# linkedin/spark-tfrecord

Measured on NVIDIA B200. Metric: TFRecord decode GB/s (1 KB Example, 64 mixed features) at 1/2/4/8 B200, higher is better.
Workload: dtype u8

## Files before the change

spark-tfrecord_b200/csrc/api_decode.inc:

```

static inline size_t align_up(size_t v, size_t a) { return (v + a - 1) / a * a; }

struct HostStats {
  FrameResult frame;
  DecodeSummary summary;
  uint32_t overflow;
  uint32_t pad[3];
};

struct K1Bufs {
  DevBuf chunks, chunk_base, first, stage, rec_off;
  uint32_t n_chunks = 0, chunk_bytes = 0;
  void release() { chunks.release(); chunk_base.release(); first.release(); stage.release(); rec_off.release(); }
};

struct PtrTables {
  void** h = nullptr; size_t cap = 0;
  DevBuf dev;
  int32_t ensure(size_t n_ptr) {
    if (cap < n_ptr) {
      if (h) cudaFreeHost(h);
      h = nullptr; cap = 0;
      CUDA_TRY(cudaHostAlloc((void**)&h, n_ptr * sizeof(void*), cudaHostAllocDefault));
      cap = n_ptr;
// ... 105 lines not shown
  unsigned long long* d_null_counts = nullptr;
  std::vector<unsigned long long> h_null_counts_tmp;
  void* host_copy = nullptr; size_t host_copy_bytes = 0;
  bool host_copy_enqueued = false;
  cudaEvent_t d2h_done = nullptr;
  bool null_counts_ready = false;
  cudaEvent_t done = nullptr;
  bool pending = false;
  Lane* lane = nullptr;
  const void* src = nullptr; size_t src_bytes = 0; int src_on_device = 0, is_final = 0;
  bool xc_tried = false;
  OutLayout lay;
  std::vector<size_t> lvl_off;
  std::vector<int32_t> uni_len;
};

static void give_event(tfr_decoder* d, cudaEvent_t e) { if (e) d->done_pool.push_back(e); }
static int32_t take_event(tfr_decoder* d, cudaEvent_t* e) {
  if (!d->done_pool.empty()) { *e = d->done_pool.back(); d->done_pool.pop_back(); return TFR_OK; }
  CUDA_TRY(cudaEventCreateWithFlags(e, cudaEventDisableTiming));
  return TFR_OK;
}

extern "C" int32_t tfr_decoder_create(const tfr_schema* schema, int32_t device, uint32_t flags, tfr_decoder** out) {
  if (!schema || !out) return fail(TFR_E_INVALID_ARG, "null argument");
  DeviceCtx* ctx = nullptr;
  int32_t rc = get_ctx(device, &ctx);
  if (rc) return rc;
  CUDA_TRY(cudaSetDevice(device));
  auto* d = new tfr_decoder;
  d->schema = *schema; d->device = device; d->flags = flags; d->ctx = ctx;
  CUDA_TRY(cudaStreamCreateWithFlags(&d->stream, cudaStreamNonBlocking));
  {
    int lo = 0, hi = 0;
    CUDA_TRY(cudaDeviceGetStreamPriorityRange(&lo, &hi));
    CUDA_TRY(cudaStreamCreateWithPriority(&d->st_k1, cudaStreamNonBlocking, getenv("TFR_NO_K1_PRIORITY") ? lo : hi));
  }
  CUDA_TRY(cudaStreamCreateWithFlags(&d->st_h2d, cudaStreamNonBlocking));
  CUDA_TRY(cudaStreamCreateWithFlags(&d->st_d2h, cudaStreamNonBlocking));
  CUDA_TRY(cudaStreamCreateWithFlags(&d->st_aux, cudaStreamNonBlocking));
  rc = d->dsch.upload(d->schema);
  if (!rc) rc = d->dsch.build_tile_consts(d->schema, ctx->d_tabs);
  if (rc) { delete d; return rc; }
  TRY(d->small.ensure(4096 + (size_t)d->schema.n_cnt * 16));
  {
    bool ok = d->schema.fields.size() <= 128 && !getenv("TFR_DISABLE_FAST");
    for (const DevField& f : d->schema.fields) if (f.depth > 1 && d->schema.record_type == TFR_RT_EXAMPLE) ok = false;
    d->fast_ok = ok;
    if (getenv("TFR_DISABLE_SPECULATION")) d->spec_state = -1;
    const size_t nv = std::max(1, d->schema.n_var);
    d->spec_len.assign(nv, -1);
    d->hist_ratio.assign(std::max(1, d->schema.n_cnt), 0.0);
    CUDA_TRY(cudaHostAlloc((void**)&d->h_uniform, nv * 4, cudaHostAllocDefault));
    TRY(d->uniform_dev.ensure(nv * 4));
    TRY(d->no_uniform_dev.ensure(nv * 4));
    CUDA_TRY(cudaMemset(d->no_uniform_dev.p, 0xff, nv * 4));
  }
  CUDA_TRY(cudaHostAlloc((void**)&d->h_stats, sizeof(HostStats), cudaHostAllocDefault));
  size_t nt = (size_t)d->schema.n_cnt * 2 + d->schema.fields.size() + 8;
  CUDA_TRY(cudaHostAlloc((void**)&d->h_totals, nt * sizeof(int64_t), cudaHostAllocDefault));
  for (Lane& L : d->lanes) {
    L.h_res_bytes = sizeof(LaneResult) + 8 * std::max<size_t>(1, d->schema.fields.size()) + 8 * std::max<size_t>(1, (size_t)d->schema.n_cnt);
    TRY(L.res.ensure(L.h_res_bytes));
    CUDA_TRY(cudaHostAlloc((void**)&L.h_res, L.h_res_bytes, cudaHostAllocDefault));
    CUDA_TRY(cudaEventCreateWithFlags(&L.ev_in, cudaEventDisableTiming));
    CUDA_TRY(cudaEventCreateWithFlags(&L.ev_k1, cudaEventDisableTiming));
    CUDA_TRY(cudaEventCreateWithFlags(&L.ev_tile, cudaEventDisableTiming));
    CUDA_TRY(cudaEventCreateWithFlags(&L.ev_frame, cudaEventDisableTiming));
    CUDA_TRY(cudaHostAlloc((void**)&L.h_frame, sizeof(FrameResult), cudaHostAllocDefault));
  }
  *out = d;
  return TFR_OK;
}
static void decoder_unref(tfr_decoder* d);
extern "C" void tfr_decoder_destroy(tfr_decoder* d) { if (d) decoder_unref(d); }
static void decoder_unref(tfr_decoder* d) {
  if (d->refs.fetch_sub(1) != 1) return;
  int prev = -1; cudaGetDevice(&prev);
  cudaSetDevice(d->device);
// ... 435 lines not shown
  return cudaSuccess;
}
static int32_t launch_bytes(DeviceCtx* ctx, const TileArgs& TA, uint32_t grid_rows, const TileGeom& g, cudaStream_t st) {
  const uint32_t grid = std::max<uint32_t>(1, (grid_rows + TILE_ROWS - 1) / TILE_ROWS);
  const size_t tiles_per_sm = std::max<size_t>(1, (size_t)233472 / (g.smem + 1024));
  static const int force = getenv("TFR_BYTES_CW") ? atoi(getenv("TFR_BYTES_CW")) : 0;
  const int cw = force ? force : tiles_per_sm >= 10 ? 4 : 8;
  cudaError_t e = cw <= 2 ? bytes_launch_one<2, 1>(ctx, TA, grid, g.smem, st) : cw <= 4 ? bytes_launch_one<4, 2>(ctx, TA, grid, g.smem, st) : bytes_launch_one<8, 4>(ctx, TA, grid, g.smem, st);
  if (e != cudaSuccess) return fail(TFR_E_CUDA, std::string("bytes kernel: ") + cudaGetErrorString(e));
  return TFR_OK;
}

static void batch_drop_outputs(tfr_batch* b) {
  tfr_decoder* d = b->dec;
  if (b->dev_fixed) { d->dev_pool.give_back(b->dev_fixed, d->stream); b->dev_fixed = nullptr; b->dev_fixed_bytes = 0; }
  if (b->dev_var) { d->dev_pool.give_back(b->dev_var, d->stream); b->dev_var = nullptr; b->dev_var_bytes = 0; }
  b->d_null_counts = nullptr; b->cols.clear(); b->null_counts_ready = false;
}

static int32_t decode_sync(tfr_decoder* d, tfr_batch* b, const void* data, size_t nbytes, int32_t data_on_device, int32_t is_final, bool allow_fast) {
  NvtxRange nvtx("tfr_decode_sync");
  cudaStream_t st = d->stream;
  const tfr_schema& S = d->schema;
  for (;;) {
    b->info = tfr_batch_info{};
    b->info.error_row = -1; b->info.error_field = -1;
    DecodeCtx C;
    C.d = d; C.b = b; C.st = st; C.nbytes = nbytes; C.nf = (uint32_t)S.fields.size(); C.lay = &b->lay; C.pt = &d->pt;
    C.verify = (d->flags & TFR_F_VERIFY_CRC) ? 1u : 0u;
    const uint32_t nf = C.nf;

    C.d_data = (const uint8_t*)data;
    if (!data_on_device && nbytes) {
      TRY(d->in.ensure(align_up(nbytes + 64, 256)));
      d->span_begin(5);
      CUDA_TRY(cudaMemcpyAsync(d->in.p, data, nbytes, cudaMemcpyHostToDevice, st));
      d->span_end(0);
      C.d_data = (const uint8_t*)d->in.p;
      data = d->in.p; data_on_device = 1;
    }
    const bool try_fast = allow_fast && d->fast_ok;
    const bool k1_verified = !try_fast || !C.verify;
    FrameResult fr{};
    fr.stop = FS_EOF;
    if (nbytes) {
      d->span_begin(0);
// ... 94 lines not shown
        TA.verify = C.verify; TA.names_bytes = names_bytes; TA.sch = d->dsch.view; TA.consts = d->dsch.d_tile_consts; TA.const_bytes = d->dsch.tile_consts_bytes;
        TA.bitmaps = C.fx + b->lay.bitmaps_off; TA.nb_stride = b->lay.nb_stride; TA.null_counts = b->d_null_counts;
        TA.fix_values = A.fix_values; TA.cnt = A.cnt; TA.src = A.src; TA.cflag = A.cflag;
        TA.uniform_len = (const int32_t*)(uniform ? d->uniform_dev.p : d->no_uniform_dev.p); TA.var_values = (void* const*)C.dt_vals; TA.flags = dflags_ptr(d);
        d->span_begin(1);
        TRY(launch_tile(d, TA, n, geom, st));
        d->span_end(1); d->pass1_launches++;
        uint32_t tflags = 0;
        if (uniform) {
          if (S.n_var) {
            d->span_begin(2);
            uniform_offsets_kernel<<<dim3(std::min<uint32_t>((n + 256) / 256, 512), S.n_var), 256, 0, st>>>((int32_t* const*)C.dt_offs, 3, (const int32_t*)d->uniform_dev.p, (uint32_t)S.n_var, n, nullptr);
            d->span_end(1);
          }
          CUDA_TRY(cudaMemcpyAsync(&d->h_stats->overflow, dovf_ptr(d), 8, cudaMemcpyDeviceToHost, st));
          CUDA_TRY(cudaStreamSynchronize(st));
          CUDA_TRY(cudaGetLastError());
          tflags = (&d->h_stats->overflow)[1];
          if (!(tflags & TF_FALLBACK)) {
            for (int a = 0; a < S.n_cnt; ++a) totals[a] = utot[a];
            TRY(finish_var_and_views(C, A, n, totals, false, false));
            done = true;
          } else {
            if (tflags & TF_SHAPE) {
              d->spec_state = 0;
              if (++d->shape_misses >= 2) d->relearn_backoff = 8;
            }
            if (b->dev_var) { d->dev_pool.give_back(b->dev_var, d->stream); b->dev_var = nullptr; b->dev_var_bytes = 0; }
            if (tflags & TF_SHAPE) {
              CUDA_TRY(cudaMemsetAsync(b->d_null_counts, 0, sizeof(unsigned long long) * std::max<uint32_t>(nf, 1), st));
              CUDA_TRY(cudaMemsetAsync(dflags_ptr(d), 0, 4, st));
              TA.uniform_len = (const int32_t*)d->no_uniform_dev.p;
              d->span_begin(1);
              TRY(launch_tile(d, TA, n, geom, st));
              d->span_end(1); d->pass1_launches++;
            }
          }
        }
        if (!done && (!uniform || (tflags & TF_SHAPE))) {
          TRY(scans_and_sync(C, A, false));
          tflags = (&d->h_stats->overflow)[1];
          if (!(tflags & TF_FALLBACK)) {
            if (d->h_stats->overflow)
              for (int a = 0; a < S.n_cnt; ++a) if (totals[a] < 0 || totals[a] > 0x7fffffffLL) return fail(TFR_E_BATCH_TOO_LARGE, "Arrow int32 offsets overflow; decode smaller blocks");
            A.flist_warp = S.record_type == TFR_RT_SEQUENCE_EXAMPLE && !getenv("TFR_DISABLE_FLIST_WARP");
            TRY(finish_var_and_views(C, A, n, totals, true, false));
            done = true;
            d->stats[3]++;
            if (d->relearn_backoff > 0) --d->relearn_backoff;
            else if (d->spec_state == 0) {
              bool ok = true, ragged = false;
              for (int v = 0; v < S.n_var && ok; ++v) {
                const DevField& fd = S.fields[S.var_field[v]];
                const int64_t c0 = totals[S.n_cnt + fd.cnt_slot];
                if (fd.n_levels == 1 && c0 > 0 && totals[fd.cnt_slot] == c0 * (int64_t)n) d->spec_len[v] = (int32_t)c0;
                else if (getenv("TFR_DISABLE_RAGGED")) ok = false;
                else if (fd.depth <= 1) { d->spec_len[v] = TILE_RAGGED; ragged = true; }
                else if (S.record_type == TFR_RT_SEQUENCE_EXAMPLE && S.n_var <= 4 && fd.elem_type != TFR_T_STRING && fd.elem_type != TFR_T_BINARY) {
                  d->spec_len[v] = TILE_RAGGED; ragged = true;
                } else ok = false;
              }
              if (ragged && ((size_t)tile_ragged_bytes((uint32_t)S.n_var, (uint32_t)S.n_cnt) > 24576 || S.n_cnt > 128)) ok = false;
              if (ok) {
                d->spec_state = 1; d->spec_ragged = ragged; d->stats[5]++;
                memcpy(d->h_uniform, d->spec_len.data(), (size_t)S.n_var * 4);
                CUDA_TRY(cudaMemcpyAsync(d->uniform_dev.p, d->h_uniform, (size_t)S.n_var * 4, cudaMemcpyHostToDevice, st));
                CUDA_TRY(cudaStreamSynchronize(st));
              }
            }
            for (int a = 0; a < S.n_cnt; ++a) d->hist_ratio[a] = used ? (double)totals[a] / (double)used : 0.0;
          }
        }
        if (done) { n_eff = n; sum.n_eff = n; if (uniform && !(tflags & TF_FALLBACK)) d->shape_misses = 0; }
      }
      if (!done && !k1_verified) {
        batch_drop_outputs(b);
        allow_fast = false;
        again = true;
      } else if (!done) {
        CUDA_TRY(cudaMemsetAsync(b->d_null_counts, 0, sizeof(unsigned long long) * std::max<uint32_t>(nf, 1), st));
        TRY(ensure_rec_off(C));
        fill_decode_args(C, A);
        const uint32_t warps = 8;
        size_t smem1 = CRC_SMEM_WORDS * 4 + (size_t)warps * ((nf + 3) & ~3u);
        uint32_t g1 = std::min<uint32_t>((n + warps - 1) / warps, (uint32_t)d->ctx->sm_count * 16);
        d->span_begin(1);
        decode_pass1_kernel<<<g1, warps * 32, smem1, st>>>(A);
        d->span_end(1); d->pass1_launches++;
        TRY(scans_and_sync(C, A, true));
// ... 9 lines not shown
      b->cols.resize(nf);
      for (uint32_t f = 0; f < nf; ++f) {
        const DevField& fd = S.fields[f];
        tfr_column c{};
        c.elem_type = fd.elem_type; c.depth = fd.depth; c.n_levels = fd.n_levels; c.value_width = fd.width;
        c.validity = C.fx + b->lay.bitmaps_off + (size_t)f * b->lay.nb_stride;
        if (fd.var_slot >= 0) { c.offsets[0] = (int32_t*)(C.fx + b->lay.off0_off[fd.var_slot]); c.n_offsets[0] = 1; }
        if (fd.fix_slot >= 0) c.values = C.fx + b->lay.fix_off[fd.fix_slot];
        for (int l = 1; l < fd.n_levels; ++l) { c.offsets[l] = c.offsets[0]; c.n_offsets[l] = 1; }
        b->cols[f] = c;
      }
    }
    if (again) continue;
    b->info.consumed_bytes = (int64_t)used;
    b->info.n_rows = n_eff;
    if (n > 0 && sum.first_err_row != 0xffffffffu) {
      b->info.error_code = -(int32_t)(sum.first_err_status & 0xff);
      b->info.error_row = sum.first_err_row;
      b->info.error_field = (int32_t)(sum.first_err_status >> 8) - 1;
    } else if (frame_err) {
      b->info.error_code = frame_err; b->info.error_row = n; b->info.error_field = -1;
    }
    if (!b->info.error_code && n > 64) { d->mean_rec_bytes = (double)fr.stop_pos / n; d->last_max_len = fr.max_len; d->last_max_tile = 0; }
    if (!b->done) TRY(take_event(d, &b->done));
    CUDA_TRY(cudaEventRecord(b->done, st));
    CUDA_TRY(cudaGetLastError());
    d->stats[0]++;
    return TFR_OK;
  }
}

static bool can_speculate(const tfr_decoder* d, const void* data, size_t nbytes, int32_t on_device, uint32_t* cap_out) {
  if (!d->fast_ok || d->spec_state != 1 || d->mean_rec_bytes < 16.0 || d->last_max_len == 0 || nbytes < 4096 || getenv("TFR_DISABLE_ASYNC")) return false;
  const double est = (double)nbytes / d->mean_rec_bytes;
  uint64_t cap = (uint64_t)(est * (1.0 + (getenv("TFR_FIXED_SLACK") ? 0.0625 : d->cap_slack))) + (getenv("TFR_FIXED_SLACK") ? 4096 : 1024);
  cap = std::min<uint64_t>(cap, nbytes / 16 + 1);
  for (int v = 0; v < d->schema.n_var; ++v) if (d->spec_len[v] >= 0 && (uint64_t)d->spec_len[v] * cap > 0x7fffffffull) return false;
  const uint32_t rg = (d->spec_ragged ? tile_ragged_bytes((uint32_t)d->schema.n_var, (uint32_t)d->schema.n_cnt) : 0u) +
                      (d->schema.record_type == TFR_RT_SEQUENCE_EXAMPLE ? tile_seq_bytes((uint32_t)d->schema.n_var, d->spec_ragged) : 0u);
  if (d->schema.record_type == TFR_RT_BYTE_ARRAY) { if (bytes_geom_for(d, d->last_max_len, true).smem > (size_t)d->ctx->max_smem_optin) return false; }
  else if (tile_geom_for(d, d->last_max_len, true, rg, d->last_max_tile).smem > (size_t)d->ctx->max_smem_optin) return false;
  *cap_out = (uint32_t)cap;
  return true;
}

static int32_t submit_async(tfr_decoder* d, Lane& L, tfr_batch* b, const void* data, size_t nbytes, int32_t on_device, int32_t is_final, uint32_t cap) {
// ... 169 lines not shown
    b->xc_tried = true;
    d->xc_batches = 64;
    const uint32_t cap = b->lay.n_alloc;
    batch_drop_outputs(b);
    b->host_copy_enqueued = false; b->host_cols.clear();
    if (b->d2h_done) CUDA_TRY(cudaEventSynchronize(b->d2h_done));
    if (b->host_copy) { d->host_pool.give_back(b->host_copy); b->host_copy = nullptr; }
    d->stats[6]++;
    TRY(submit_async(d, L, b, b->src, b->src_bytes, 1, b->is_final, cap));
    return resolve(b);
  }
  d->stats[2]++;
  if (fr.n_records > b->lay.n_alloc) d->cap_slack = 0.0625;
  const bool unlearned = (r.flags & TF_SHAPE) && d->spec_state == 1;
  if (r.flags & TF_SHAPE) {
    d->spec_state = 0;
    if (++d->shape_misses >= 2) d->relearn_backoff = 8;
  }
  batch_drop_outputs(b);
  b->host_copy_enqueued = false; b->host_cols.clear();
  if (b->d2h_done) CUDA_TRY(cudaEventSynchronize(b->d2h_done));
  if (b->host_copy) { d->host_pool.give_back(b->host_copy); b->host_copy = nullptr; }
  TRY(decode_sync(d, b, b->src, b->src_bytes, 1, b->is_final, true));
  if (b->src == L.in.p) CUDA_TRY(cudaEventSynchronize(b->done));
  if (unlearned && b->info.error_code && d->spec_state == 0) { d->spec_state = 1; if (d->shape_misses > 0) --d->shape_misses; d->relearn_backoff = 0; }
  return TFR_OK;
}

static int32_t lane_make_free(tfr_decoder* d, Lane& L) {
  if (L.pending) TRY(resolve(L.pending));
  if (L.orphan_done) {
    CUDA_TRY(cudaEventSynchronize(L.orphan_done));
    give_event(d, L.orphan_done); L.orphan_done = nullptr;
    const LaneResult r = *L.h_res;
    if (r.flags & TF_FALLBACK) d->stats[2]++;
    if (r.flags & TF_SHAPE) { d->spec_state = 0; if (++d->shape_misses >= 2) d->relearn_backoff = 8; }
    else if (!(r.flags & TF_FALLBACK) && r.frame.n_records > 64) { d->mean_rec_bytes = (double)r.frame.stop_pos / r.frame.n_records; d->last_max_len = r.frame.max_len; d->last_max_tile = r.max_tile; }
  }
  return TFR_OK;
}

extern "C" int32_t tfr_decode_submit(tfr_decoder* d, const void* data, size_t nbytes, int32_t data_on_device, int32_t is_final, tfr_batch** out) {
  if (!d || !out || (nbytes && !data)) return fail(TFR_E_INVALID_ARG, "null argument");
  if (nbytes >= (1ull << 31)) return fail(TFR_E_BATCH_TOO_LARGE, "tfr_decode: a batch must be smaller than 2 GiB; split the file at record boundaries");
  NvtxRange nvtx("tfr_decode_submit");
  std::lock_guard<std::recursive_mutex> lk(d->mu);
// ... 176 lines not shown
```

spark-tfrecord_b200/csrc/tile.cuh:

```cuda
#pragma once
#include "common.cuh"
#include "decode.cuh"

#define TILE_ROWS 32
#ifndef TILE_PARSE_WARPS
#define TILE_PARSE_WARPS 12
#endif
#ifndef TILE_CRC_WARPS
#define TILE_CRC_WARPS 3
#endif
#define TILE_THREADS ((TILE_PARSE_WARPS + TILE_CRC_WARPS) * 32)
#ifndef TILE_MIN_CTAS
#define TILE_MIN_CTAS 3
#endif
#define TILE_TPL_WORDS 5

struct FieldTemplate {
  uint32_t words[TILE_TPL_WORDS];
  uint32_t mask[TILE_TPL_WORDS];
  uint16_t n_words;
  uint16_t klen;
  uint32_t kind;
};

// ... 15 lines not shown
  uint32_t const_bytes;
  uint8_t* bitmaps;
  uint32_t nb_stride;
  unsigned long long* null_counts;
  void* const* fix_values;
  uint32_t* cnt;
  uint32_t* src;
  uint8_t* cflag;
  const int32_t* uniform_len;
  uint32_t ragged;
  uint32_t n_cnt;
  uint32_t* ticket;
  uint32_t* lb_flag;
  uint32_t* lb_agg;
  unsigned long long* lb_pre;
  const unsigned long long* cap;
  unsigned long long* totals;
  int32_t* const* offs;
  const int32_t* var_field;
  void* const* var_values;
  uint32_t* flags;
};

enum { TF_FALLBACK = 1u, TF_SHAPE = 2u, TF_OVERFLOW = 4u, TF_XCODE = 8u };
#define TILE_RAGGED (-2)

__device__ __forceinline__ uint32_t smem_u32(const void* p) { return (uint32_t)__cvta_generic_to_shared(p); }
__device__ __forceinline__ void mbar_init(uint64_t* bar, uint32_t count) {
  asm volatile("mbarrier.init.shared::cta.b64 [%0], %1;" ::"r"(smem_u32(bar)), "r"(count));
}
__device__ __forceinline__ void mbar_expect_tx(uint64_t* bar, uint32_t bytes) {
  asm volatile("mbarrier.arrive.expect_tx.shared::cta.b64 _, [%0], %1;" ::"r"(smem_u32(bar)), "r"(bytes) : "memory");
}
__device__ __forceinline__ void bulk_g2s(void* dst, const void* src, uint32_t bytes, uint64_t* bar) {
  asm volatile("cp.async.bulk.shared::cluster.global.mbarrier::complete_tx::bytes [%0], [%1], %2, [%3];" ::"r"(smem_u32(dst)),
               "l"(src), "r"(bytes), "r"(smem_u32(bar))
               : "memory");
}
__device__ __forceinline__ void mbar_wait(uint64_t* bar, uint32_t phase) {
  uint32_t ok;
  do {
    asm volatile(
        "{\n"
        ".reg .pred p;\n"
        "mbarrier.try_wait.parity.shared::cta.b64 p, [%1], %2;\n"
        "selp.u32 %0, 1, 0, p;\n"
        "}\n"
        : "=r"(ok)
// ... 29 lines not shown
  }
  __device__ __forceinline__ int32_t i8(uint32_t o) const {
    int32_t v;
    asm("ld.shared.s8 %0, [%1];" : "=r"(v) : "r"(s + o));
    return v;
  }
  __device__ __forceinline__ uint4 w128(uint32_t o) const {
    uint4 v;
    asm("ld.shared.v4.u32 {%0, %1, %2, %3}, [%4];" : "=r"(v.x), "=r"(v.y), "=r"(v.z), "=r"(v.w) : "r"(s + o));
    return v;
  }
  __device__ __forceinline__ uint32_t w32(uint32_t o) const {
    uint32_t v;
    asm("ld.shared.u32 %0, [%1];" : "=r"(v) : "r"(s + o));
    return v;
  }
};
__device__ __forceinline__ uint32_t t_u32(const Tile& t, uint32_t o) {
  const uint32_t a = o & ~3u;
  uint32_t sh = (o & 3u) * 8;
  uint32_t lo = t.w32(a);
  return sh ? __funnelshift_r(lo, t.w32(a + 4), sh) : lo;
}
__device__ __forceinline__ bool t_len(const Tile& t, uint32_t& p, uint32_t end, uint32_t& v) {
  if (p >= end) return false;
  uint32_t b = t.u8(p++);
  if (b < 0x80) { v = b; return true; }
  uint32_t r = b & 0x7f;
#pragma unroll 1
  for (int sh = 7; sh < 35; sh += 7) {
    if (p >= end) return false;
    b = t.u8(p++);
    r |= (b & 0x7f) << sh;
    if (b < 0x80) { v = r; return (int32_t)r >= 0; }
  }
  return false;
}

__device__ __forceinline__ void t_copy_out(const Tile& t, uint32_t src, uint8_t* dst, uint32_t l) {
  uint32_t i = 0;
  const uint32_t mis = (uint32_t)(reinterpret_cast<uintptr_t>(dst) & 3u);
  if (mis) for (const uint32_t h = min(l, 4u - mis); i < h; ++i) dst[i] = (uint8_t)t.u8(src + i);
  for (; i + 4 <= l; i += 4) *reinterpret_cast<uint32_t*>(dst + i) = t_u32(t, src + i);
  for (; i < l; ++i) dst[i] = (uint8_t)t.u8(src + i);
}

// ... 13 lines not shown
  const uint32_t x = (c ^ b) & 0xff;
  return (c >> 8) ^ g[416 + (x & 31)] ^ g[448 + (x >> 5)];
}
__device__ __forceinline__ uint32_t crc_chunks(const uint32_t* g, const Tile& t, uint32_t o, uint32_t k, uint32_t c) {
#pragma unroll 2
  for (uint32_t i = 0; i < k; ++i) {
    const uint4 v = t.w128(o + 16 * i);
    c = crc_fold8(g, c, v.x, v.y);
    c = crc_fold8(g, c, v.z, v.w);
  }
  return c;
}

#define TILE_SEEN_BYTES (512u + 128u + 16u)
#define TILE_CRC_BYTES (2048u + 2048u)
__host__ __device__ inline uint32_t tile_schema_smem(uint32_t nf, uint32_t names_bytes) {
  return ((nf * (uint32_t)sizeof(DevField) + 15u) & ~15u) + ((nf * (uint32_t)sizeof(FieldTemplate) + 15u) & ~15u) + ((names_bytes + 15u) & ~15u);
}
__host__ __device__ inline uint32_t tile_const_bytes(uint32_t nf, uint32_t names_bytes) { return TILE_CRC_BYTES + TILE_SEEN_BYTES + tile_schema_smem(nf, names_bytes); }
__host__ __device__ inline uint32_t tile_ragged_bytes(uint32_t n_var, uint32_t n_cnt) { return (n_var + n_cnt) * 128u + n_cnt * 4u + n_cnt * 8u + 16u + 16u + 96u; }
#define TILE_SQ_STEPS 128u
__host__ __device__ inline uint32_t tile_seq_bytes(uint32_t n_var, bool with_steps = false) { return n_var * 256u + 16u + (with_steps ? n_var * TILE_SQ_STEPS * 32u : 0u); }
__host__ __device__ inline uint32_t tile_smem_bytes(uint32_t nf, uint32_t names_bytes, uint32_t tile_cap, uint32_t ragged_bytes = 0) {
  return 16 + tile_const_bytes(nf, names_bytes) + tile_cap + 64 + ragged_bytes;
}

template <bool SEQ, bool RG, int PW, int CW, bool XC>
__global__ void __launch_bounds__((PW + CW) * 32, (PW >= 16 ? 2 : PW >= 12 ? TILE_MIN_CTAS : 8)) decode_tile_kernel(TileArgs A) {
  extern __shared__ __align__(128) uint8_t smem_raw[];
  uint64_t* bar = reinterpret_cast<uint64_t*>(smem_raw);
  uint32_t* s8 = reinterpret_cast<uint32_t*>(smem_raw + 16);
  uint32_t* sseen = reinterpret_cast<uint32_t*>(smem_raw + 16 + TILE_CRC_BYTES);
  const uint32_t nf = (uint32_t)A.sch.n_fields;
  uint8_t* sbase = smem_raw + 16 + TILE_CRC_BYTES + TILE_SEEN_BYTES;
  DevField* sfields = reinterpret_cast<DevField*>(sbase);
  FieldTemplate* stpl = reinterpret_cast<FieldTemplate*>(sbase + ((nf * (uint32_t)sizeof(DevField) + 15u) & ~15u));
  uint8_t* snames = sbase + ((nf * (uint32_t)sizeof(DevField) + 15u) & ~15u) + ((nf * (uint32_t)sizeof(FieldTemplate) + 15u) & ~15u);
  uint8_t* tile_b = sbase + tile_schema_smem(nf, A.names_bytes);
  const uint32_t lane = threadIdx.x & 31, wid = threadIdx.x >> 5;

  uint32_t* rg_src = reinterpret_cast<uint32_t*>(tile_b + A.tile_cap + 64);
  uint32_t* rg_cnt = rg_src + (uint32_t)A.sch.n_var * 32u;
  uint32_t* rg_tot = rg_cnt + A.n_cnt * 32u;
  unsigned long long* rg_base = reinterpret_cast<unsigned long long*>(rg_tot + ((A.n_cnt + 1u) & ~1u) + 24u);
  uint32_t* rg_tile = rg_tot + ((A.n_cnt + 1u) & ~1u);
  uint32_t* sq_cnt = reinterpret_cast<uint32_t*>(tile_b + A.tile_cap + 64 + (RG ? tile_ragged_bytes((uint32_t)A.sch.n_var, A.n_cnt) : 0u));
  uint8_t* sq_tab = reinterpret_cast<uint8_t*>(sq_cnt + (uint32_t)A.sch.n_var * 64u + 4u);
  if (SEQ) for (uint32_t i = threadIdx.x; i < (uint32_t)A.sch.n_var * 64u; i += (PW + CW) * 32) sq_cnt[i] = 0u;
  uint32_t tile = blockIdx.x;
  if (RG) {
    if (threadIdx.x == 0) { rg_tile[0] = atomicAdd(A.ticket, 1u); rg_tile[1] = 0u; rg_tile[2 + PW] = 0u; }
    for (uint32_t i = threadIdx.x; i < A.n_cnt * 32u; i += ((PW + CW) * 32)) rg_cnt[i] = 0u;
    __syncthreads();
    tile = rg_tile[0];
  }
  const uint32_t row0 = tile * TILE_ROWS;
  uint32_t n_rows = A.n;
  if (A.n_dev) {
    n_rows = *A.n_dev;
    if (n_rows > A.n) {
      if (tile == 0 && threadIdx.x == 0) atomicOr(A.flags, TF_OVERFLOW | TF_FALLBACK);
// ... 20 lines not shown
  uint32_t tile_tot;
  uint32_t rbase = warp_excl_scan_u32(active ? ((stride + 111u) & ~127u) + 16u : 0u, tile_tot);
  uint32_t tile_need = tile_tot;
  if (A.slot) { rbase = lane * A.slot; tile_need = __any_sync(FULLMASK, stride > A.slot) ? 0xffffffffu : 0u; }
  if (threadIdx.x == 0 && A.tile_max) atomicMax(A.tile_max, tile_tot);
  if (tile_need > A.tile_cap) {
    if (threadIdx.x == 0) {
      atomicOr(A.flags, TF_FALLBACK);
      if (RG) {
        for (uint32_t a = 0; a < A.n_cnt; ++a) A.lb_pre[(size_t)tile * ((A.n_cnt + 3u) & ~3u) + a] = 0ull;
        __threadfence();
        st_release_u32(&A.lb_flag[tile], 2u);
      }
    }
    return;
  }
  if (wid == 0) {
    if (lane == 0) {
      mbar_init(bar, 1);
      asm volatile("fence.mbarrier_init.release.cluster;" ::: "memory");
    }
    const uint32_t total = __reduce_add_sync(FULLMASK, bulk_bytes);
    if (lane == 0) {
      mbar_expect_tx(bar, total + A.const_bytes);
      bulk_g2s(smem_raw + 16, A.consts, A.const_bytes, bar);
    }
    __syncwarp();
    if (bulk_bytes) bulk_g2s(tile_b + rbase + (b_lo - g_lo), base + b_lo, bulk_bytes, bar);
    if (active) {
      uint8_t* sl = tile_b + rbase;
      const uint32_t e1 = min(b_lo, lim);
      if (b_lo > g_lo) for (uint32_t i = mis; i < e1; ++i) sl[i - g_lo] = base[i];
      if (b_hi < g_lo + cbytes) for (uint32_t i = max(b_hi, e1); i < lim; ++i) sl[i - g_lo] = base[i];
    }
  }
  __syncthreads();
  mbar_wait(bar, 0);

  const uint32_t len = flen - 16;
  const uint32_t pay = rbase + head + 12;
  const uint32_t end = pay + len;
  const uint32_t g0 = (off - head) - rbase;
  Tile T;
  T.b = tile_b;
  asm volatile("mov.u32 %0, %1;" : "=r"(T.s) : "r"(smem_u32(tile_b)) : "memory");

  if (wid >= PW) {
    const uint32_t cw = wid - PW;
// ... 33 lines not shown
    return;
  }

  bool bad = false;
  uint32_t skip = wid;
  uint32_t shape_bad = 0;
  unsigned long long seen_lo = 0, seen_hi = 0;
  if (active) {
    uint32_t p = pay, L = 0;
    uint32_t cend = end, fl_start = end, fl_end = end;
    if (len < 2 || T.u8(p) != 0x0A) bad = true;
    else {
      ++p;
      if (!t_len(T, p, end, L) || end - p < L) bad = true;
      else if (!SEQ) { if (p + L != end) bad = true; }
      else {
        cend = p + L;
        uint32_t q = cend, L2 = 0;
        if (q >= end || T.u8(q) != 0x12) bad = true;
        else { ++q; if (!t_len(T, q, end, L2) || q + L2 != end) bad = true; else { fl_start = q; fl_end = end; } }
      }
    }
    uint32_t next_f = wid;
    while (!bad && p < cend) {
      for (bool wide = true; wide;) {
        wide = false;
        while (skip && p < cend) {
          const int32_t b1 = T.i8(p + 1);
          if (b1 < 0) { wide = true; break; }
          p += 2u + (uint32_t)b1;
          --skip;
        }
        if (wide) {
          uint32_t q = p + 1, el;
          if (!t_len(T, q, cend, el)) { bad = true; break; }
          p = q + el;
          --skip;
        }
      }
      if (bad || p >= cend) break;
      skip = PW - 1;
      uint32_t eend, kind, llen;
      int f = -1;
      bool located = false;
      if (next_f < nf && stpl[next_f].n_words) {
        const FieldTemplate& tp = stpl[next_f];
        const uint32_t klen = tp.klen;
        const uint32_t ab = p & ~3u, sh = (p & 3u) * 8;
        uint32_t aw[TILE_TPL_WORDS + 1];
#pragma unroll
        for (int w = 0; w <= TILE_TPL_WORDS; ++w) aw[w] = T.w32(ab + 4 * w);
        uint32_t diff = 0, u0 = 0;
#pragma unroll
        for (int w = 0; w < TILE_TPL_WORDS; ++w) {
          const uint32_t u = __funnelshift_r(aw[w], aw[w + 1], sh);
          if (w == 0) u0 = u;
          diff |= (u ^ tp.words[w]) & tp.mask[w];
        }
        const uint32_t elen = (u0 >> 8) & 0xff, vl = T.u8(p + 5 + klen), ll = T.u8(p + 7 + klen);
        if (diff == 0 && elen < 0x80 && elen == klen + 4 + vl && vl == ll + 2 && p + 2 + elen <= cend) {
          f = (int)next_f; eend = p + 2 + elen; located = true;
          kind = tp.kind; llen = ll;
          p += klen + 8;
        }
      }
      if (!located) {
        uint32_t elen, klen, vlen;
        if (T.u8(p) != 0x0A) { bad = true; break; }
        ++p;
        if (!t_len(T, p, cend, elen) || cend - p < elen) { bad = true; break; }
        eend = p + elen;
        if (p >= eend || T.u8(p) != 0x0A) { bad = true; break; }
        ++p;
        if (!t_len(T, p, eend, klen) || eend - p < klen) { bad = true; break; }
        const uint32_t key = p;
        p += klen;
        if (p >= eend || T.u8(p) != 0x12) { bad = true; break; }
        ++p;
        if (!t_len(T, p, eend, vlen) || p + vlen != eend) { bad = true; break; }
        uint32_t hi = 0;
        for (uint32_t i = 0; i < klen; ++i) hi |= T.u8(key + i);
        if (hi >= 0x80 && !utf8_valid(T.b + key, klen)) { bad = true; break; }
        uint32_t h = name_hash(T.b + key, klen);
        uint32_t slot = h & (uint32_t)A.sch.ht_mask;
        for (;;) {
          int cand = A.sch.ht[slot];
          if (cand < 0) break;
          if (sfields[cand].hash == h && sfields[cand].name_len == klen) {
            const uint8_t* nm = snames + sfields[cand].name_off;
            uint32_t diff = 0;
            for (uint32_t i = 0; i < klen; ++i) diff |= T.u8(key + i) ^ nm[i];
            if (diff == 0) { f = cand; break; }
          }
          slot = (slot + 1) & (uint32_t)A.sch.ht_mask;
// ... 36 lines not shown
            for (uint32_t i = 0; i < bl; ++i) acc |= T.u8(p + i);
            if (acc >= 0x80 && !utf8_valid(T.b + p, bl)) {
              if (RG && XC && A.uniform_len[fd->var_slot] == TILE_RAGGED) xcode = true;
              else {
                if (RG && A.uniform_len[fd->var_slot] == TILE_RAGGED) atomicOr(A.flags, TF_XCODE);
                bad = true; break;
              }
            }
          }
          if (n == 0) { first_off = lp + g0; first_len = bl; first_data = p; }
          ++n; total += bl;
          p += bl;
        }
        if (bad) break;
        if (fd) {
          if (fd->depth == 0) {
            if (n == 0) { bad = true; break; }
            const int32_t ul = A.uniform_len[fd->var_slot];
            if (RG && ul == TILE_RAGGED) {
              rg_src[fd->var_slot * 32 + lane] = first_data | (xcode ? 0x80000000u : 0u);
              rg_cnt[fd->cnt_slot * 32 + lane] = first_len;
              if (xcode) atomicOr(&sseen[161], 1u);
            } else if (ul >= 0) {
              if ((uint32_t)ul != first_len) shape_bad = 1;
              else {
                uint8_t* dst = reinterpret_cast<uint8_t*>(A.var_values[fd->var_slot]) + (size_t)row * (uint32_t)ul;
                if ((ul & 15) == 0) {
                  for (uint32_t i = 0; i < (uint32_t)ul; i += 16) {
                    uint4 v;
                    v.x = t_u32(T, first_data + i); v.y = t_u32(T, first_data + i + 4); v.z = t_u32(T, first_data + i + 8); v.w = t_u32(T, first_data + i + 12);
                    *reinterpret_cast<uint4*>(dst + i) = v;
                  }
                } else for (uint32_t i = 0; i < (uint32_t)ul; ++i) dst[i] = T.u8(first_data + i);
              }
            } else {
              A.cnt[(size_t)fd->cnt_slot * A.n + row] = first_len;
              A.src[(size_t)fd->var_slot * A.n + row] = first_off;
              A.cflag[(size_t)fd->var_slot * A.n + row] = CF_CANON;
            }
          } else {
            if (RG && A.uniform_len[fd->var_slot] == TILE_RAGGED) {
              if (xcode) atomicOr(&sseen[161], 1u);
              rg_src[fd->var_slot * 32 + lane] = body | (xcode ? 0x80000000u : 0u);
              rg_cnt[fd->cnt_slot * 32 + lane] = n;
              rg_cnt[(fd->cnt_slot + 1) * 32 + lane] = total;
            } else {
            A.cnt[(size_t)fd->cnt_slot * A.n + row] = n;
            A.cnt[(size_t)(fd->cnt_slot + 1) * A.n + row] = total;
            A.src[(size_t)fd->var_slot * A.n + row] = body + g0;
            A.cflag[(size_t)fd->var_slot * A.n + row] = CF_CANON;
            }
          }
        }
      } else {
        uint32_t plen = 0, pk = p;
        if (llen != 0) {
          if (T.u8(p) != 0x0A) { bad = true; break; }
          ++p;
          if (!t_len(T, p, eend, plen) || p + plen != eend) { bad = true; break; }
          pk = p;
        }
        uint32_t n;
        uint64_t v0 = 0;
        if (kind == K_FLOAT) {
          if (plen & 3) { bad = true; break; }
          n = plen >> 2;
        } else {
          n = 0;
          if (plen >= 1 && plen <= 8) {
            const uint32_t w0 = t_u32(T, pk), w1 = plen > 4 ? t_u32(T, pk + 4) : 0u;
            unsigned long long x = ((unsigned long long)w1 << 32) | w0;
            const unsigned long long live = ~0ull >> (64 - 8 * plen);
            const unsigned long long term = ~x & 0x8080808080808080ull & live;
            if (!((term >> (8 * plen - 1)) & 1)) { bad = true; break; }
            n = (uint32_t)__popcll(term);
            const uint32_t k0 = (uint32_t)__ffsll((long long)term);
            x &= (~0ull >> (64 - k0)) & 0x7f7f7f7f7f7f7f7full;
            x = ((x & 0x7f007f007f007f00ull) >> 1) | (x & 0x007f007f007f007full);
            x = ((x & 0x3fff00003fff0000ull) >> 2) | (x & 0x00003fff00003fffull);
            x = ((x & 0x0fffffff00000000ull) >> 4) | (x & 0x000000000fffffffull);
            v0 = x;
          } else {
            uint32_t run = 0;
            for (uint32_t i = 0; i < plen; ++i) {
              uint32_t b = T.u8(pk + i);
              if (n == 0) v0 |= (uint64_t)(b & 0x7f) << (7 * run);
              if (b & 0x80) { if (++run >= 10) { bad = true; break; } } else { ++n; run = 0; }
            }
            if (bad || run) { bad = true; break; }
          }
        }
        if (fd) {
          if (fd->depth == 0) {
            if (n == 0) { bad = true; break; }
            void* vp = A.fix_values[fd->fix_slot];
            if (kind == K_FLOAT) {
              uint32_t bits = t_u32(T, pk);
              if (fd->elem_type == TFR_T_FLOAT32) reinterpret_cast<uint32_t*>(vp)[row] = bits;
              else reinterpret_cast<double*>(vp)[row] = (double)__uint_as_float(bits);
            } else {
              if (fd->elem_type == TFR_T_INT64) reinterpret_cast<int64_t*>(vp)[row] = (int64_t)v0;
              else reinterpret_cast<int32_t*>(vp)[row] = (int32_t)(uint32_t)v0;
            }
          } else {
            const int32_t ul = A.uniform_len[fd->var_slot];
            if (RG && ul == TILE_RAGGED) {
              rg_src[fd->var_slot * 32 + lane] = pk;
              rg_cnt[fd->cnt_slot * 32 + lane] = n;
            } else if (ul >= 0) {
              if ((uint32_t)ul != n) shape_bad = 1;
              else if (kind == K_FLOAT) {
                if (fd->elem_type == TFR_T_FLOAT32) {
                  uint32_t* dst = reinterpret_cast<uint32_t*>(A.var_values[fd->var_slot]) + (size_t)row * n;
                  if ((n & 3) == 0) {
                    for (uint32_t i = 0; i < n; i += 4) {
                      uint4 v;
                      v.x = t_u32(T, pk + 4 * i); v.y = t_u32(T, pk + 4 * i + 4); v.z = t_u32(T, pk + 4 * i + 8); v.w = t_u32(T, pk + 4 * i + 12);
                      *reinterpret_cast<uint4*>(dst + i) = v;
                    }
                  } else for (uint32_t i = 0; i < n; ++i) dst[i] = t_u32(T, pk + 4 * i);
                } else {
                  double* dst = reinterpret_cast<double*>(A.var_values[fd->var_slot]) + (size_t)row * n;
                  for (uint32_t i = 0; i < n; ++i) dst[i] = (double)__uint_as_float(t_u32(T, pk + 4 * i));
                }
              } else {
                uint32_t q = pk;
                for (uint32_t e = 0; e < n; ++e) {
                  uint64_t v = 0; uint32_t sh = 0;
                  for (;;) { uint32_t b = T.u8(q++); v |= (uint64_t)(b & 0x7f) << sh; sh += 7; if (b < 0x80) break; }
                  if (fd->elem_type == TFR_T_INT64) reinterpret_cast<int64_t*>(A.var_values[fd->var_slot])[(size_t)row * n + e] = (int64_t)v;
                  else reinterpret_cast<int32_t*>(A.var_values[fd->var_slot])[(size_t)row * n + e] = (int32_t)(uint32_t)v;
                }
              }
            } else {
              A.cnt[(size_t)fd->cnt_slot * A.n + row] = n;
              A.src[(size_t)fd->var_slot * A.n + row] = pk + g0;
              A.cflag[(size_t)fd->var_slot * A.n + row] = CF_CANON;
            }
          }
        }
      }
      p = eend;
// ... 351 lines not shown
  {
    const bool row_bad = (sseen[160] >> lane) & 1u;
    uint32_t all[4];
#pragma unroll
    for (int k = 0; k < 4; ++k) all[k] = sseen[lane * 4 + k];
    const uint32_t act_mask = __ballot_sync(FULLMASK, active);
    for (uint32_t f = wid; f < nf; f += PW) {
      const uint32_t wsel = f < 32 ? all[0] : f < 64 ? all[1] : f < 96 ? all[2] : all[3];
      const bool present = (wsel >> (f & 31)) & 1;
      const uint32_t m = __ballot_sync(FULLMASK, present && active);
      if (SEQ && active && present && sfields[f].depth == 2 && A.cnt) {
        const DevField& fd = sfields[f];
        A.cnt[(size_t)(fd.cnt_slot + 1) * A.n + row] = sq_cnt[(fd.var_slot * 32 + lane) * 2];
        if (fd.n_levels == 3) A.cnt[(size_t)(fd.cnt_slot + 2) * A.n + row] = sq_cnt[(fd.var_slot * 32 + lane) * 2 + 1];
      }
      if (active && !present && sfields[f].elem_type != TFR_T_NULL) {
        const DevField& fd = sfields[f];
        if (!fd.nullable) bad = true;
        if (fd.fix_slot >= 0) {
          void* vp = A.fix_values[fd.fix_slot];
          if (fd.width == 8) reinterpret_cast<uint64_t*>(vp)[row] = 0; else reinterpret_cast<uint32_t*>(vp)[row] = 0;
        } else if (fd.var_slot >= 0) {
          const int32_t ul = A.uniform_len[fd.var_slot];
          if (ul > 0 && !row_bad) shape_bad = 1;
          else if (ul == -1) for (int l = 0; l < fd.n_levels; ++l) A.cnt[(size_t)(fd.cnt_slot + l) * A.n + row] = 0;
        }
      }
      if (lane == 0) {
        reinterpret_cast<uint32_t*>(A.bitmaps + (size_t)f * A.nb_stride)[tile] = m;
        const uint32_t nulls = __popc(act_mask & ~m);
        if (nulls) atomicAdd(&A.null_counts[f], (unsigned long long)nulls);
      }
    }
  }
  if (bad) atomicOr(A.flags, TF_FALLBACK);
  if (shape_bad) atomicOr(A.flags, TF_SHAPE | TF_FALLBACK);
}

__global__ void uniform_offsets_kernel(int32_t* const* __restrict__ offs, uint32_t stride, const int32_t* __restrict__ uniform_len, uint32_t n_var,
                                       uint32_t n, const uint32_t* __restrict__ n_dev) {
  const uint32_t v = blockIdx.y;
  if (v >= n_var) return;
  if (n_dev) { const uint32_t m = *n_dev; if (m > n) return; n = m; }
  const int32_t L = uniform_len[v];
  if (L < 0) return;
  int32_t* o = offs[v * stride];
  for (uint32_t i = blockIdx.x * blockDim.x + threadIdx.x; i <= n; i += gridDim.x * blockDim.x) o[i] = (int32_t)(i * (uint32_t)L);
}
```

Measured before the change: 1133.

## Add speculative feature jump table to skip fixed-size entries in tile decoder

Once uniform lengths are learned, the host builds a per-field jump table holding each entry's predicted encoded length and prefix sums. The table is uploaded alongside the uniform lengths and bulk-copied into shared memory. Each warp then skips runs of predictable feature entries with one add instead of parsing every varint header. Mispredicted entry lengths raise a new TF_JUMP flag that forces fallback and turns the table off. Bulk float and bytes copies also switch to a funnel-shift helper that reads each tile word once, at the cost of an extra null-count download and sync when speculation is relearned.

New measurement: 1162 (median of 6 runs). +2.6%, better.

```diff
diff --git a/spark-tfrecord_b200/csrc/api_decode.inc b/spark-tfrecord_b200/csrc/api_decode.inc
--- a/spark-tfrecord_b200/csrc/api_decode.inc
+++ b/spark-tfrecord_b200/csrc/api_decode.inc
@@ -151,6 +151,50 @@
   return TFR_OK;
 }
 
+static size_t uniform_buf_bytes(const tfr_schema& S) {
+  return std::max<size_t>(4, tile_jump_off((uint32_t)S.n_var) + tile_jump_bytes((uint32_t)S.fields.size()));
+}
+static uint32_t varint_bytes(uint32_t v) { uint32_t n = 1; while (v >= 0x80) { v >>= 7; ++n; } return n; }
+static void fill_jump_table(const tfr_schema& S, const int32_t* len, const unsigned long long* nulls, int32_t* buf) {
+  const uint32_t nf = (uint32_t)S.fields.size();
+  std::vector<uint32_t> el(nf + 1, 0), pre(nf + 1, 0), fs(nf + 1, 0xffffu), re(nf + 1, 0xffffu);
+  uint32_t k = 0;
+  bool armed = nulls != nullptr;
+  for (uint32_t f = 0; f < nf; ++f) {
+    const DevField& fd = S.fields[f];
+    if (S.record_type == TFR_RT_SEQUENCE_EXAMPLE && fd.depth == 2) continue;
+    if (armed && (fd.elem_type == TFR_T_NULL || nulls[f])) armed = false;
+    const int32_t ul = fd.var_slot >= 0 ? len[fd.var_slot] : -1;
+    uint32_t list = 0;
+    if (armed && ul > 0 && fd.n_levels == 1 && fd.kind == K_FLOAT && fd.depth == 1) list = 1 + varint_bytes(4u * ul) + 4u * ul;
+    if (armed && ul >= 0 && fd.n_levels == 1 && fd.kind == K_BYTES && fd.depth == 0) list = 1 + varint_bytes(ul) + ul;
+    if (list) {
+      const uint32_t value = 1 + varint_bytes(list) + list;
+      const uint32_t elen = 1 + varint_bytes(fd.name_len) + fd.name_len + 1 + varint_bytes(value) + value;
+      el[k] = 1 + varint_bytes(elen) + elen;
+    }
+    ++k;
+  }
+  for (uint32_t i = 0; i < nf; ++i) pre[i + 1] = pre[i] + el[i];
+  for (uint32_t i = nf; i-- > 0;) {
+    if (el[i]) { fs[i] = i; re[i] = el[i + 1] ? re[i + 1] : i + 1; }
+    else { fs[i] = fs[i + 1]; re[i] = re[i + 1]; }
+  }
+  uint32_t* tab = reinterpret_cast<uint32_t*>(reinterpret_cast<uint8_t*>(buf) + tile_jump_off((uint32_t)S.n_var));
+  for (uint32_t i = 0; i <= nf; ++i) {
+    tab[4 * i + 0] = fs[i] | re[i] << 16;
+    tab[4 * i + 1] = fs[i] == 0xffffu ? 0u : pre[re[i]] - pre[i];
+    tab[4 * i + 2] = pre[i];
+    tab[4 * i + 3] = el[i];
+  }
+}
+static int32_t jumps_off(tfr_decoder* d) {
+  const size_t off = tile_jump_off((uint32_t)d->schema.n_var);
+  CUDA_TRY(cudaMemcpyAsync((uint8_t*)d->uniform_dev.p + off, (const uint8_t*)d->no_uniform_dev.p + off, tile_jump_bytes((uint32_t)d->schema.fields.size()),
+                           cudaMemcpyDeviceToDevice, d->stream));
+  return TFR_OK;
+}
+
 extern "C" int32_t tfr_decoder_create(const tfr_schema* schema, int32_t device, uint32_t flags, tfr_decoder** out) {
   if (!schema || !out) return fail(TFR_E_INVALID_ARG, "null argument");
   DeviceCtx* ctx = nullptr;
@@ -180,10 +224,14 @@
     const size_t nv = std::max(1, d->schema.n_var);
     d->spec_len.assign(nv, -1);
     d->hist_ratio.assign(std::max(1, d->schema.n_cnt), 0.0);
-    CUDA_TRY(cudaHostAlloc((void**)&d->h_uniform, nv * 4, cudaHostAllocDefault));
-    TRY(d->uniform_dev.ensure(nv * 4));
-    TRY(d->no_uniform_dev.ensure(nv * 4));
-    CUDA_TRY(cudaMemset(d->no_uniform_dev.p, 0xff, nv * 4));
+    const size_t ub = uniform_buf_bytes(d->schema);
+    CUDA_TRY(cudaHostAlloc((void**)&d->h_uniform, ub, cudaHostAllocDefault));
+    TRY(d->uniform_dev.ensure(ub));
+    TRY(d->no_uniform_dev.ensure(ub));
+    for (size_t v = 0; v < nv; ++v) d->h_uniform[v] = -1;
+    fill_jump_table(d->schema, d->h_uniform, nullptr, d->h_uniform);
+    CUDA_TRY(cudaMemcpy(d->no_uniform_dev.p, d->h_uniform, ub, cudaMemcpyHostToDevice));
+    CUDA_TRY(cudaMemcpy(d->uniform_dev.p, d->h_uniform, ub, cudaMemcpyHostToDevice));
   }
   CUDA_TRY(cudaHostAlloc((void**)&d->h_stats, sizeof(HostStats), cudaHostAllocDefault));
   size_t nt = (size_t)d->schema.n_cnt * 2 + d->schema.fields.size() + 8;
@@ -665,6 +713,7 @@
   NvtxRange nvtx("tfr_decode_sync");
   cudaStream_t st = d->stream;
   const tfr_schema& S = d->schema;
+  bool jump_miss = false;
   for (;;) {
     b->info = tfr_batch_info{};
     b->info.error_row = -1; b->info.error_field = -1;
@@ -805,6 +854,7 @@
             TRY(finish_var_and_views(C, A, n, totals, false, false));
             done = true;
           } else {
+            if ((tflags & (TF_JUMP | TF_SHAPE)) == TF_JUMP) jump_miss = true;
             if (tflags & TF_SHAPE) {
               d->spec_state = 0;
               if (++d->shape_misses >= 2) d->relearn_backoff = 8;
@@ -847,7 +897,11 @@
               if (ok) {
                 d->spec_state = 1; d->spec_ragged = ragged; d->stats[5]++;
                 memcpy(d->h_uniform, d->spec_len.data(), (size_t)S.n_var * 4);
-                CUDA_TRY(cudaMemcpyAsync(d->uniform_dev.p, d->h_uniform, (size_t)S.n_var * 4, cudaMemcpyHostToDevice, st));
+                b->h_null_counts_tmp.resize(std::max<uint32_t>(nf, 1));
+                CUDA_TRY(cudaMemcpyAsync(b->h_null_counts_tmp.data(), b->d_null_counts, sizeof(unsigned long long) * nf, cudaMemcpyDeviceToHost, st));
+                CUDA_TRY(cudaStreamSynchronize(st));
+                fill_jump_table(S, d->spec_len.data(), b->h_null_counts_tmp.data(), d->h_uniform);
+                CUDA_TRY(cudaMemcpyAsync(d->uniform_dev.p, d->h_uniform, uniform_buf_bytes(S), cudaMemcpyHostToDevice, st));
                 CUDA_TRY(cudaStreamSynchronize(st));
               }
             }
@@ -903,6 +957,7 @@
       b->info.error_code = frame_err; b->info.error_row = n; b->info.error_field = -1;
     }
     if (!b->info.error_code && n > 64) { d->mean_rec_bytes = (double)fr.stop_pos / n; d->last_max_len = fr.max_len; d->last_max_tile = 0; }
+    if (jump_miss && !b->info.error_code) TRY(jumps_off(d));
     if (!b->done) TRY(take_event(d, &b->done));
     CUDA_TRY(cudaEventRecord(b->done, st));
     CUDA_TRY(cudaGetLastError());
@@ -1118,6 +1173,7 @@
   if (b->d2h_done) CUDA_TRY(cudaEventSynchronize(b->d2h_done));
   if (b->host_copy) { d->host_pool.give_back(b->host_copy); b->host_copy = nullptr; }
   TRY(decode_sync(d, b, b->src, b->src_bytes, 1, b->is_final, true));
+  if ((r.flags & (TF_JUMP | TF_SHAPE)) == TF_JUMP && !b->info.error_code) TRY(jumps_off(d));
   if (b->src == L.in.p) CUDA_TRY(cudaEventSynchronize(b->done));
   if (unlearned && b->info.error_code && d->spec_state == 0) { d->spec_state = 1; if (d->shape_misses > 0) --d->shape_misses; d->relearn_backoff = 0; }
   return TFR_OK;
diff --git a/spark-tfrecord_b200/csrc/tile.cuh b/spark-tfrecord_b200/csrc/tile.cuh
--- a/spark-tfrecord_b200/csrc/tile.cuh
+++ b/spark-tfrecord_b200/csrc/tile.cuh
@@ -61,8 +61,11 @@
   uint32_t* flags;
 };
 
-enum { TF_FALLBACK = 1u, TF_SHAPE = 2u, TF_OVERFLOW = 4u, TF_XCODE = 8u };
+enum { TF_FALLBACK = 1u, TF_SHAPE = 2u, TF_OVERFLOW = 4u, TF_XCODE = 8u, TF_JUMP = 16u };
 #define TILE_RAGGED (-2)
+
+__host__ __device__ inline uint32_t tile_jump_off(uint32_t n_var) { return (n_var * 4u + 15u) & ~15u; }
+__host__ __device__ inline uint32_t tile_jump_bytes(uint32_t nf) { return (nf + 1u) * 16u; }
 
 __device__ __forceinline__ uint32_t smem_u32(const void* p) { return (uint32_t)__cvta_generic_to_shared(p); }
 __device__ __forceinline__ void mbar_init(uint64_t* bar, uint32_t count) {
@@ -138,6 +141,15 @@
   uint32_t lo = t.w32(a);
   return sh ? __funnelshift_r(lo, t.w32(a + 4), sh) : lo;
 }
+__device__ __forceinline__ void t_copy_u4(const Tile& t, uint32_t src, uint4* dst, uint32_t n16) {
+  const uint32_t a = src & ~3u, sh = (src & 3u) * 8;
+  uint32_t lo = t.w32(a);
+  for (uint32_t i = 0; i < n16; ++i) {
+    const uint32_t b = a + 16 * i, w1 = t.w32(b + 4), w2 = t.w32(b + 8), w3 = t.w32(b + 12), w4 = t.w32(b + 16);
+    dst[i] = make_uint4(__funnelshift_r(lo, w1, sh), __funnelshift_r(w1, w2, sh), __funnelshift_r(w2, w3, sh), __funnelshift_r(w3, w4, sh));
+    lo = w4;
+  }
+}
 __device__ __forceinline__ bool t_len(const Tile& t, uint32_t& p, uint32_t end, uint32_t& v) {
   if (p >= end) return false;
   uint32_t b = t.u8(p++);
@@ -197,7 +209,7 @@
 #define TILE_SQ_STEPS 128u
 __host__ __device__ inline uint32_t tile_seq_bytes(uint32_t n_var, bool with_steps = false) { return n_var * 256u + 16u + (with_steps ? n_var * TILE_SQ_STEPS * 32u : 0u); }
 __host__ __device__ inline uint32_t tile_smem_bytes(uint32_t nf, uint32_t names_bytes, uint32_t tile_cap, uint32_t ragged_bytes = 0) {
-  return 16 + tile_const_bytes(nf, names_bytes) + tile_cap + 64 + ragged_bytes;
+  return 16 + tile_const_bytes(nf, names_bytes) + tile_jump_bytes(nf) + tile_cap + 64 + ragged_bytes;
 }
 
 template <bool SEQ, bool RG, int PW, int CW, bool XC>
@@ -211,7 +223,8 @@
   DevField* sfields = reinterpret_cast<DevField*>(sbase);
   FieldTemplate* stpl = reinterpret_cast<FieldTemplate*>(sbase + ((nf * (uint32_t)sizeof(DevField) + 15u) & ~15u));
   uint8_t* snames = sbase + ((nf * (uint32_t)sizeof(DevField) + 15u) & ~15u) + ((nf * (uint32_t)sizeof(FieldTemplate) + 15u) & ~15u);
-  uint8_t* tile_b = sbase + tile_schema_smem(nf, A.names_bytes);
+  uint8_t* const jtab = sbase + tile_schema_smem(nf, A.names_bytes);
+  uint8_t* tile_b = jtab + tile_jump_bytes(nf);
   const uint32_t lane = threadIdx.x & 31, wid = threadIdx.x >> 5;
 
   uint32_t* rg_src = reinterpret_cast<uint32_t*>(tile_b + A.tile_cap + 64);
@@ -278,8 +291,9 @@
     }
     const uint32_t total = __reduce_add_sync(FULLMASK, bulk_bytes);
     if (lane == 0) {
-      mbar_expect_tx(bar, total + A.const_bytes);
+      mbar_expect_tx(bar, total + A.const_bytes + tile_jump_bytes(nf));
       bulk_g2s(smem_raw + 16, A.consts, A.const_bytes, bar);
+      bulk_g2s(jtab, reinterpret_cast<const uint8_t*>(A.uniform_len) + tile_jump_off((uint32_t)A.sch.n_var), tile_jump_bytes(nf), bar);
     }
     __syncwarp();
     if (bulk_bytes) bulk_g2s(tile_b + rbase + (b_lo - g_lo), base + b_lo, bulk_bytes, bar);
@@ -359,24 +373,38 @@
       }
     }
     uint32_t next_f = wid;
+    uint32_t ei = 0;
+    const uint32_t jt = 0u - tile_jump_bytes(nf);
     while (!bad && p < cend) {
-      for (bool wide = true; wide;) {
-        wide = false;
-        while (skip && p < cend) {
-          const int32_t b1 = T.i8(p + 1);
-          if (b1 < 0) { wide = true; break; }
-          p += 2u + (uint32_t)b1;
-          --skip;
-        }
-        if (wide) {
-          uint32_t q = p + 1, el;
-          if (!t_len(T, q, cend, el)) { bad = true; break; }
-          p = q + el;
-          --skip;
-        }
-      }
+      const uint32_t t = ei + skip;
+      while (ei < t && p < cend) {
+        const uint4 J = T.w128(jt + 16u * min(ei, nf));
+        const uint32_t wend = min(J.x & 0xffffu, t);
+        for (bool wide = true; wide;) {
+          wide = false;
+          while (ei < wend && p < cend) {
+            const int32_t b1 = T.i8(p + 1);
+            if (b1 < 0) { wide = true; break; }
+            p += 2u + (uint32_t)b1;
+            ++ei;
+          }
+          if (wide) {
+            uint32_t q = p + 1, el;
+            if (!t_len(T, q, cend, el)) { bad = true; break; }
+            p = q + el;
+            ++ei;
+          }
+        }
+        if (bad || ei < wend || ei == t || p >= cend) break;
+        const uint32_t re = J.x >> 16;
+        if (re <= t) { p += J.y; ei = re; }
+        else { p += T.w32(jt + 16u * t + 8u) - J.z; ei = t; }
+      }
+      skip = t - ei;
       if (bad || p >= cend) break;
       skip = PW - 1;
+      const uint32_t jlen = T.w32(jt + 16u * min(ei, nf) + 12u);
+      ++ei;
       uint32_t eend, kind, llen;
       int f = -1;
       bool located = false;
@@ -398,15 +426,18 @@
         if (diff == 0 && elen < 0x80 && elen == klen + 4 + vl && vl == ll + 2 && p + 2 + elen <= cend) {
           f = (int)next_f; eend = p + 2 + elen; located = true;
           kind = tp.kind; llen = ll;
+          if (jlen && 2 + elen != jlen) shape_bad |= 2u;
           p += klen + 8;
         }
       }
       if (!located) {
         uint32_t elen, klen, vlen;
+        const uint32_t p0 = p;
         if (T.u8(p) != 0x0A) { bad = true; break; }
         ++p;
         if (!t_len(T, p, cend, elen) || cend - p < elen) { bad = true; break; }
         eend = p + elen;
+        if (jlen && eend - p0 != jlen) shape_bad |= 2u;
         if (p >= eend || T.u8(p) != 0x0A) { bad = true; break; }
         ++p;
         if (!t_len(T, p, eend, klen) || eend - p < klen) { bad = true; break; }
@@ -489,15 +520,11 @@
               rg_cnt[fd->cnt_slot * 32 + lane] = first_len;
               if (xcode) atomicOr(&sseen[161], 1u);
             } else if (ul >= 0) {
-              if ((uint32_t)ul != first_len) shape_bad = 1;
+              if ((uint32_t)ul != first_len) shape_bad |= 1u;
               else {
                 uint8_t* dst = reinterpret_cast<uint8_t*>(A.var_values[fd->var_slot]) + (size_t)row * (uint32_t)ul;
                 if ((ul & 15) == 0) {
-                  for (uint32_t i = 0; i < (uint32_t)ul; i += 16) {
-                    uint4 v;
-                    v.x = t_u32(T, first_data + i); v.y = t_u32(T, first_data + i + 4); v.z = t_u32(T, first_data + i + 8); v.w = t_u32(T, first_data + i + 12);
-                    *reinterpret_cast<uint4*>(dst + i) = v;
-                  }
+                  t_copy_u4(T, first_data, reinterpret_cast<uint4*>(dst), (uint32_t)ul >> 4);
                 } else for (uint32_t i = 0; i < (uint32_t)ul; ++i) dst[i] = T.u8(first_data + i);
               }
             } else {
@@ -535,7 +562,9 @@
         } else {
           n = 0;
           if (plen >= 1 && plen <= 8) {
-            const uint32_t w0 = t_u32(T, pk), w1 = plen > 4 ? t_u32(T, pk + 4) : 0u;
+            const uint32_t a = pk & ~3u, sh = (pk & 3u) * 8;
+            const uint32_t x0 = T.w32(a), x1 = (sh || plen > 4) ? T.w32(a + 4) : 0u, x2 = (sh && plen > 4) ? T.w32(a + 8) : 0u;
+            const uint32_t w0 = __funnelshift_r(x0, x1, sh), w1 = plen > 4 ? __funnelshift_r(x1, x2, sh) : 0u;
             unsigned long long x = ((unsigned long long)w1 << 32) | w0;
             const unsigned long long live = ~0ull >> (64 - 8 * plen);
             const unsigned long long term = ~x & 0x8080808080808080ull & live;
@@ -575,16 +604,12 @@
               rg_src[fd->var_slot * 32 + lane] = pk;
               rg_cnt[fd->cnt_slot * 32 + lane] = n;
             } else if (ul >= 0) {
-              if ((uint32_t)ul != n) shape_bad = 1;
+              if ((uint32_t)ul != n) shape_bad |= 1u;
               else if (kind == K_FLOAT) {
                 if (fd->elem_type == TFR_T_FLOAT32) {
                   uint32_t* dst = reinterpret_cast<uint32_t*>(A.var_values[fd->var_slot]) + (size_t)row * n;
                   if ((n & 3) == 0) {
-                    for (uint32_t i = 0; i < n; i += 4) {
-                      uint4 v;
-                      v.x = t_u32(T, pk + 4 * i); v.y = t_u32(T, pk + 4 * i + 4); v.z = t_u32(T, pk + 4 * i + 8); v.w = t_u32(T, pk + 4 * i + 12);
-                      *reinterpret_cast<uint4*>(dst + i) = v;
-                    }
+                    t_copy_u4(T, pk, reinterpret_cast<uint4*>(dst), n >> 2);
                   } else for (uint32_t i = 0; i < n; ++i) dst[i] = t_u32(T, pk + 4 * i);
                 } else {
                   double* dst = reinterpret_cast<double*>(A.var_values[fd->var_slot]) + (size_t)row * n;
@@ -982,7 +1007,7 @@
           if (fd.width == 8) reinterpret_cast<uint64_t*>(vp)[row] = 0; else reinterpret_cast<uint32_t*>(vp)[row] = 0;
         } else if (fd.var_slot >= 0) {
           const int32_t ul = A.uniform_len[fd.var_slot];
-          if (ul > 0 && !row_bad) shape_bad = 1;
+          if (ul > 0 && !row_bad) shape_bad |= 1u;
           else if (ul == -1) for (int l = 0; l < fd.n_levels; ++l) A.cnt[(size_t)(fd.cnt_slot + l) * A.n + row] = 0;
         }
       }
@@ -994,7 +1019,8 @@
     }
   }
   if (bad) atomicOr(A.flags, TF_FALLBACK);
-  if (shape_bad) atomicOr(A.flags, TF_SHAPE | TF_FALLBACK);
+  if (shape_bad & 1u) atomicOr(A.flags, TF_SHAPE | TF_FALLBACK);
+  if (shape_bad & 2u) atomicOr(A.flags, TF_JUMP | TF_FALLBACK);
 }
 
 __global__ void uniform_offsets_kernel(int32_t* const* __restrict__ offs, uint32_t stride, const int32_t* __restrict__ uniform_len, uint32_t n_var,
```
